# godai0519/BayesianNetwork

Measured on AMD Instinct MI355X. Metric: edge-messages/sec to BP convergence, higher is better.
Workload: dtype f64; 1 GPU; 316x316 2D-grid BN, k=4, 99856 nodes, 199080 edges (BASELINE.json configs[2]), 998 evidence nodes, eps=0.001; parallelism=1 GPU

## Files before the change

### bayesiannetwork_amd/csrc/bn_resident.hip

```cpp
#include "bn_tiles.hpp"

namespace bnmi {

#define RLX_AGENT __ATOMIC_RELAXED, __HIP_MEMORY_SCOPE_AGENT

#ifdef BN_TILE_CLOCK
#define RSTAMP(k, iter, lane_, wave_)                                                              \
    do {                                                                                           \
        if ((iter) == 5 && (lane_) == 0) g_tile_clock[blockIdx.x * kResidentWaves + (wave_)][k] = wall_clock64(); \
    } while (0)
constexpr int kRunClockStamps = 8;
static __device__ unsigned long long g_run_clock[kTileClockTiles][kRunClockStamps];
#define RUNSTAMP(k, lane_, wave_)                                                                   \
    do {                                                                                           \
        if ((lane_) == 0) g_run_clock[blockIdx.x * kResidentWaves + (wave_)][k] = wall_clock64();   \
    } while (0)
#else
#define RSTAMP(k, iter, lane_, wave_) ((void)0)
#define RUNSTAMP(k, lane_, wave_) ((void)0)
#endif

typedef unsigned u32x4 __attribute__((ext_vector_type(4)));
__device__ __forceinline__ double2_t ld_rec(__amdgpu_buffer_rsrc_t r, int64_t idx2) {
    return __builtin_bit_cast(double2_t, __builtin_amdgcn_raw_buffer_load_b128(r, int(idx2) * 16, 0, 16));
}
__device__ __forceinline__ void st_rec(__amdgpu_buffer_rsrc_t r, int64_t idx2, double2_t v) {
    __builtin_amdgcn_raw_buffer_store_b128(__builtin_bit_cast(u32x4, v), r, int(idx2) * 16, 0, 16);
}
__device__ __forceinline__ double2_t ld_rec_sys(__amdgpu_buffer_rsrc_t r, int64_t idx2) {
    return __builtin_bit_cast(double2_t, __builtin_amdgcn_raw_buffer_load_b128(r, int(idx2) * 16, 0, 17));
}
__device__ __forceinline__ void st_rec_sys(__amdgpu_buffer_rsrc_t r, int64_t idx2, double2_t v) {
    __builtin_amdgcn_raw_buffer_store_b128(__builtin_bit_cast(u32x4, v), r, int(idx2) * 16, 0, 17);
}
__device__ __forceinline__ void drain_stores() { asm volatile("s_waitcnt vmcnt(0)" ::: "memory"); }

__device__ __forceinline__ void pin_here(double& x) { asm volatile("" : "+v"(x)); }

#ifndef BN_RES_PRIO
#define BN_RES_PRIO 6
#endif
template <int SCHED, int G>
__device__ __forceinline__ bool prio_segment(int wave) {
    if constexpr (SCHED == 2 || (SCHED == 3 && G < 2)) {
        if (((wave >> 2) & 1) != (G & 1)) __builtin_amdgcn_s_setprio(1);
        else __builtin_amdgcn_s_setprio(0);
        return true;
    } else if constexpr (SCHED == 4) {
        __builtin_amdgcn_s_setprio(3 - G);
        return true;
    } else if constexpr (SCHED == 5 && G != 2) {
        __builtin_amdgcn_s_setprio(G == 0 ? 2 : G == 1 ? 1 : 0);
        return true;
    } else if constexpr (SCHED == 6 && G != 2) {
        if (G == 3 && (wave & 4) == 0) __builtin_amdgcn_s_setprio(0);
        else __builtin_amdgcn_s_setprio(G == 0 ? 3 : G == 1 ? 2 : 1);
        return true;
    }
    return false;
}

struct BlockShared {
    unsigned long long slot[kResidentMaxSets][kResidentWaves];
    int verdict[kResidentMaxSets];
    unsigned long long t_arrive;
    int skew_ticks;
    int arrived[kResidentMaxSets];
    int poll_it[kResidentMaxSets];
    int ver[kResidentMaxSets];
};
enum : int { kGoOn = 0, kConverged = 1, kCapped = 2, kAbort = 3 };

__device__ __forceinline__ double residual_of(unsigned long long bits) {
    const double r = __longlong_as_double((long long)bits);
    return r < DBL_MIN ? DBL_MIN : r;
}
__device__ __forceinline__ int verdict_of(const ResidentArgs& a, double r, int n_done) {
    if (r < a.eps) return kConverged;
    if (a.max_sweeps > 0 && n_done >= a.max_sweeps) return kCapped;
    return kGoOn;
}

__device__ __forceinline__ unsigned long long granule(unsigned gen, unsigned half) { return ((unsigned long long)gen << 32) | half; }

__device__ __forceinline__ void arrive(const ResidentArgs& a, BlockShared& sh, int set, int it, int s, double wres, int lane,
                                       int wave) {
    const unsigned long long bits = wave_umax((unsigned long long)__double_as_longlong(wres));
    if (lane == 0) sh.slot[set][wave] = bits;
    RSTAMP(3, it, lane, wave);
    drain_stores();
    RSTAMP(4, it, lane, wave);
    __syncthreads();
    RSTAMP(5, it, lane, wave);
    if (threadIdx.x == 0) {
        unsigned long long m = 0;
        for (int w = 0; w < a.waves; ++w) m = sh.slot[set][w] > m ? sh.slot[set][w] : m;
        ResidentSync* sy = a.sync + set;
        if (a.n_tile_blocks == 1) {
            sy->res[it] = m;
            sh.verdict[set] = verdict_of(a, residual_of(m), s + 1);
        } else {
            const unsigned gen = a.gen_base + unsigned(it) + 1u;
            unsigned long long* g = (a.direct != 0 && (it & 1)) ? sy->blk_odd[blockIdx.x] : sy->blk[blockIdx.x];
            const unsigned long long now = wall_clock64();
            sh.t_arrive = now;
            __hip_atomic_store(g, granule(gen, unsigned(m >> 32)), RLX_AGENT);
            __hip_atomic_store(g + 1, ((now & 0xffffull) << 48) | ((unsigned long long)(gen & 0xffffu) << 32) | unsigned(m), RLX_AGENT);
        }
    }
}

__device__ __forceinline__ void arrive_batch(const ResidentArgs& a, BlockShared& sh, int set, int it, int s, double wres, int lane, int wave) {
    const unsigned long long bits = wave_umax((unsigned long long)__double_as_longlong(wres));
    if (lane == 0) sh.slot[set][wave] = bits;
    RSTAMP(3, it, lane, wave);
    drain_stores();
    RSTAMP(4, it, lane, wave);
    if (lane == 0) {
        const int before = __hip_atomic_fetch_add(&sh.arrived[set], 1, __ATOMIC_ACQ_REL, __HIP_MEMORY_SCOPE_WORKGROUP);
        if (before == a.waves - 1) {
            __hip_atomic_store(&sh.arrived[set], 0, __ATOMIC_RELAXED, __HIP_MEMORY_SCOPE_WORKGROUP);
            __builtin_amdgcn_fence(__ATOMIC_ACQUIRE, "workgroup");
            unsigned long long m = 0;
            for (int w = 0; w < a.waves; ++w) m = sh.slot[set][w] > m ? sh.slot[set][w] : m;
            ResidentSync* sy = a.sync + set;
            if (a.n_tile_blocks == 1) {
                sy->res[it] = m;
                __hip_atomic_store(&sh.ver[set], it << 2 | verdict_of(a, residual_of(m), s + 1), __ATOMIC_RELEASE, __HIP_MEMORY_SCOPE_WORKGROUP);
            } else {
                const unsigned gen = a.gen_base + unsigned(it) + 1u;
                unsigned long long* g = sy->blk[blockIdx.x];
                const unsigned long long now = wall_clock64();
                __hip_atomic_store(g, granule(gen, unsigned(m >> 32)), RLX_AGENT);
                __hip_atomic_store(g + 1, ((now & 0xffffull) << 48) | ((unsigned long long)(gen & 0xffffu) << 32) | unsigned(m), RLX_AGENT);
            }
        }
    }
    RSTAMP(5, it, lane, wave);
}

template <class Pred>
__device__ __forceinline__ bool poll_until(const ResidentArgs& a, Pred&& pred) {
    const unsigned long long t0 = wall_clock64();
    for (unsigned n = 1;; ++n) {
        if (pred()) return true;
        if ((n & 7u) == 0) {
            if (__hip_atomic_load(&a.sync->abort, RLX_AGENT) != 0) return false;
            if (wall_clock64() - t0 > a.timeout_ticks) {
                if (pred()) return true;
                __hip_atomic_store(&a.sync->abort, 1u, RLX_AGENT);
                return false;
            }
        }
        __builtin_amdgcn_s_sleep(1);
    }
}

__device__ __forceinline__ bool sweep_granules(const unsigned long long* tbl, int lane, int nb, unsigned gen, unsigned long long& acc,
                                               unsigned own16 = 0u, int* late_out = nullptr) {
    static_assert(kResidentMaxBlocks == 4 * kWave, "four pairs per lane cover the table");
    const unsigned voff = unsigned(lane) * 16u;
    u32x4 r0, r1, r2, r3;
    if (nb <= kWave)
        asm volatile("global_load_dwordx4 %0, %1, %2 sc1\n\ts_waitcnt vmcnt(0)" : "=&v"(r0) : "v"(voff), "s"(tbl) : "memory");
    else
        asm volatile("global_load_dwordx4 %0, %4, %5 sc1\n\t"
                     "global_load_dwordx4 %1, %4, %5 offset:1024 sc1\n\t"
                     "global_load_dwordx4 %2, %4, %5 offset:2048 sc1\n\t"
                     "global_load_dwordx4 %3, %4, %5 offset:3072 sc1\n\t"
                     "s_waitcnt vmcnt(0)"
                     : "=&v"(r0), "=&v"(r1), "=&v"(r2), "=&v"(r3) : "v"(voff), "s"(tbl) : "memory");
    bool mine = true;
    acc = 0;
    int late = 0;
    auto take = [&](const u32x4& r, int blk) {
        if (blk < nb) {
            mine = mine && r.y == gen && (r.w & 0xffffu) == (gen & 0xffffu);
            const unsigned long long v = (unsigned long long)r.x << 32 | r.z;
            acc = v > acc ? v : acc;
            const int d = int(short((r.w >> 16) - own16));
            late = d > late ? d : late;
        }
    };
    take(r0, lane);
    if (nb > kWave) { take(r1, lane + kWave); take(r2, lane + 2 * kWave); take(r3, lane + 3 * kWave); }
    if (late_out) *late_out = late;
    return mine;
}

__device__ __forceinline__ int wait_verdict(const ResidentArgs& a, BlockShared& sh, int set, int it) {
    if (a.direct != 0 && a.n_tile_blocks > 1) {
        if (threadIdx.x < kWave) {
            int lane = int(threadIdx.x);
            asm volatile("" : "+v"(lane));
            ResidentSync* sy = a.sync + set;
            const unsigned gen = a.gen_base + unsigned(it) + 1u;
            const int nb = a.n_tile_blocks;
            const unsigned long long* tbl = (it & 1) ? &sy->blk_odd[0][0] : &sy->blk[0][0];
            unsigned long long m = 0;
            const unsigned long long t_arr = sh.t_arrive;
            const unsigned own16 = unsigned(t_arr) & 0xffffu;
            if (a.first_poll_delay >= 0) {
                const unsigned long long first_at = t_arr + (unsigned long long)(sh.skew_ticks + a.first_poll_delay);
                while (wall_clock64() < first_at) __builtin_amdgcn_s_sleep(1);
            }
            int late = 0;
            const bool ok = poll_until(a, [&] { return __all(sweep_granules(tbl, lane, nb, gen, m, own16, &late)) != 0; });
            m = wave_umax(m);
            {
                int mx = late;
#pragma unroll
                for (int off = 32; off >= 1; off >>= 1) { const int o = __shfl_xor(mx, off, kWave); mx = o > mx ? o : mx; }
                if (lane == 0) sh.skew_ticks = ok ? (mx < 400 ? mx : 400) : 0;
            }
            if (lane == 0) {
                if (blockIdx.x == 0 && ok) __hip_atomic_store(&sy->res[it], m, RLX_AGENT);
                sh.verdict[set] = ok ? verdict_of(a, residual_of(m), a.sweep_begin + it + 1) : kAbort;
            }
        }
        __syncthreads();
        return sh.verdict[set];
    }
    if (threadIdx.x == 0 && a.n_tile_blocks > 1) {
        ResidentSync* sy = a.sync + set;
        const unsigned gen = a.gen_base + unsigned(it) + 1u;
        const int groups = a.n_tile_blocks < 8 ? a.n_tile_blocks : 8;
        const int g = blockIdx.x % groups;
        unsigned word = 0;
        const bool ok = poll_until(a, [&] {
            word = __hip_atomic_load(&sy->grp[g].gen, RLX_AGENT);
            return (word & 0x3fffffffu) >= gen;
        });
        sh.verdict[set] = ok ? int(word >> 30) : kAbort;
    }
    __syncthreads();
    return sh.verdict[set];
}

__device__ __forceinline__ int wait_verdict_batch(const ResidentArgs& a, BlockShared& sh, int set, int it, int lane) {
    int out = __hip_atomic_load(&sh.ver[set], __ATOMIC_ACQUIRE, __HIP_MEMORY_SCOPE_WORKGROUP);
    if ((out >> 2) == it) return out & 3;
    int before = it;
    if (lane == 0) before = __hip_atomic_fetch_max(&sh.poll_it[set], it, __ATOMIC_ACQ_REL, __HIP_MEMORY_SCOPE_WORKGROUP);
    if (__builtin_amdgcn_readfirstlane(before) < it && a.n_tile_blocks > 1) {
        if (lane == 0) {
            ResidentSync* sy = a.sync + set;
            const unsigned gen = a.gen_base + unsigned(it) + 1u;
            const int groups = a.n_tile_blocks < 8 ? a.n_tile_blocks : 8;
            const int g = blockIdx.x % groups;
            unsigned word = 0;
            const bool ok = poll_until(a, [&] {
                word = __hip_atomic_load(&sy->grp[g].gen, RLX_AGENT);
                return (word & 0x3fffffffu) >= gen;
            });
            __hip_atomic_store(&sh.ver[set], it << 2 | (ok ? int(word >> 30) : kAbort), __ATOMIC_RELEASE, __HIP_MEMORY_SCOPE_WORKGROUP);
        }
    }
    const unsigned long long t0 = wall_clock64();
    for (unsigned n = 1; ((out = __hip_atomic_load(&sh.ver[set], __ATOMIC_ACQUIRE, __HIP_MEMORY_SCOPE_WORKGROUP)) >> 2) != it; ++n) {
        if ((n & 63u) == 0 && wall_clock64() - t0 > 2 * a.timeout_ticks) {
            __hip_atomic_store(&a.sync->abort, 1u, RLX_AGENT);
            return kAbort;
        }
        __builtin_amdgcn_s_sleep(1);
    }
    return out & 3;
}

__device__ __forceinline__ void resident_service(const ResidentArgs& a, int lane) {
    if (a.direct != 0) return;
    const int nb = a.n_tile_blocks;
    const int groups = nb < 8 ? nb : 8;
    unsigned active = a.set_mask;
    for (int it = 0; it < a.budget; ++it) {
        const unsigned gen = a.gen_base + unsigned(it) + 1u;
        for (int set = 0; set < a.n_sets; ++set) {
            if (((active >> set) & 1u) == 0) continue;
            ResidentSync* sy = a.sync + set;
            unsigned long long m = 0;
            if (!poll_until(a, [&] { return __all(sweep_granules(&sy->blk[0][0], lane, nb, gen, m)) != 0; }))
                return;
            m = wave_umax(m);
            const int verdict = verdict_of(a, residual_of(m), a.sweep_begin + it + 1);
            if (lane == 0) {
                __hip_atomic_store(&sy->res[it], m, RLX_AGENT);
                asm volatile("s_waitcnt vmcnt(0)" ::: "memory");
                const unsigned word = gen | (unsigned(verdict) << 30);
                for (int q = 0; q < groups; ++q) __hip_atomic_store(&sy->grp[q].gen, word, RLX_AGENT);
            }
            if (verdict != kGoOn) active &= ~(1u << set);
        }
        if (active == 0) break;
    }
}

template <bool BATCH, class Phase, class Finalize>
__device__ __forceinline__ bool resident_drive(const ResidentArgs& a, BlockShared& sh, int lane, int wave, Phase&& phase,
                                               Finalize&& finalize) {
    unsigned active = BATCH ? a.set_mask : 1u;
    const int n_sets = BATCH ? a.n_sets : 1;
    for (int it = 0; it <= a.budget; ++it) {
        const int s = a.sweep_begin + it;
        for (int set = 0; set < n_sets; ++set) {
            if (((active >> set) & 1u) == 0) continue;
            int v = kGoOn;
            RSTAMP(0, it, lane, wave);
            if (it > 0) {
                if (BATCH && a.direct == 0) v = wait_verdict_batch(a, sh, set, it - 1, lane);
                else v = wait_verdict(a, sh, set, it - 1);
                if (v == kAbort) return false;
            }
            RSTAMP(1, it, lane, wave);
            if (v != kGoOn || it == a.budget) {
                const int done = v != kGoOn ? v : 0;
                RUNSTAMP(4, lane, wave);
                finalize(set, s, done, true);
                RUNSTAMP(5, lane, wave);
                if (blockIdx.x == 0 && wave == 0) {
                    const ResidentSync* sy = a.sync + set;
                    double* hist = a.b.res_hist + int64_t(set) * a.res_hist_stride;
                    int q0 = lane;
                    asm volatile("" : "+v"(q0));
                    for (int q = q0; q < it; q += kWave)
                        if (a.sweep_begin + q < a.b.res_cap)
                            hist[a.sweep_begin + q] = residual_of(__hip_atomic_load(&sy->res[q], RLX_AGENT));
                    if (lane == 0) {
                        Ctl* hc = a.host_ctl + set;
                        hc->last_res = it > 0 ? residual_of(__hip_atomic_load(&sy->res[it - 1], RLX_AGENT)) : 0.0;
                        hc->n_sweeps = s;
                        hc->run_id = a.run_id;
                        hc->done = done;
                    }
                }
                active &= ~(1u << set);
                continue;
            }
            const double wres = phase(set, s);
            if (BATCH && a.direct == 0) arrive_batch(a, sh, set, it, s, wres, lane, wave);
            else arrive(a, sh, set, it, s, wres, lane, wave);
            RSTAMP(6, it, lane, wave);
            if (it == 0) RUNSTAMP(3, lane, wave);
        }
        if (active == 0) break;
    }
    return true;
}

template <bool BATCH>
__device__ __forceinline__ bool resident_idle(const ResidentArgs& a, BlockShared& sh, int lane, int wave) {
    return resident_drive<BATCH>(a, sh, lane, wave, [](int, int) { return 0.0; }, [](int, int, int, bool) {});
}

#define RLX_SYS __ATOMIC_RELAXED, __HIP_MEMORY_SCOPE_SYSTEM
template <bool SHARD>
__device__ __forceinline__ unsigned long long flow_load(const unsigned long long* p) {
    if constexpr (SHARD) return __hip_atomic_load(p, RLX_SYS);
    else return __hip_atomic_load(p, RLX_AGENT);
}
template <bool SHARD>
__device__ __forceinline__ void flow_store(unsigned long long* p, unsigned long long v) {
    if constexpr (SHARD) __hip_atomic_store(p, v, RLX_SYS);
    else __hip_atomic_store(p, v, RLX_AGENT);
}
__device__ __forceinline__ unsigned long long* flow_slot(FlowSync* f, int nranks, int par, int slot) {
    return reinterpret_cast<unsigned long long*>(f + 1) + (size_t(par) * nranks * kFlowSlotsPerRank + slot) * 2;
}

template <bool SHARD>
__device__ __forceinline__ void flow_raise_abort(const ResidentArgs& a, unsigned where = 0) {
    const unsigned long long w = (unsigned long long)(a.gen_base + 1u) | ((unsigned long long)kFlowAbort << 32);
    for (int q = 0; q < 8; ++q) flow_store<SHARD>(&a.flow->verdict[q].word, w);
    if constexpr (SHARD) {
        for (int r = 0; r < a.b.nranks; ++r)
            if (r != a.b.rank)
                for (int q = 0; q < 8; ++q) flow_store<true>(&a.peers[r].flow->verdict[q].word, w);
    }
    __hip_atomic_store(a.host_abort, 0x80000000u | where, __ATOMIC_RELAXED, __HIP_MEMORY_SCOPE_SYSTEM);
}

template <bool SHARD>
__device__ __forceinline__ unsigned flow_wait(const ResidentArgs& a, int tile, int it, int lane, int& n_it) {
    n_it = 0;
    if (it == 0) return kFlowGoOn;
    FlowSync* f = a.flow;
    const int32_t* nbr_list = a.nbr + int64_t(tile) * a.nbr_chunks * kWave + lane;
    int round = 0;
    int nbr = nbr_list[0];
    const unsigned long long* vword = &f->verdict[blockIdx.x & 7].word;
    const unsigned want_nb = a.gen_base + unsigned(it);
    const unsigned want_v = a.gen_base + unsigned(it) - 1u;
    unsigned long long t0 = 0;
    for (unsigned polls = 0;; ++polls) {
        bool nb_ok = true;
        if (nbr >= 0) nb_ok = unsigned(flow_load<SHARD>(flow_slot(f, a.b.nranks, (it - 1) & 1, nbr)) >> 32) == want_nb;
        if (__all(nb_ok) && round + 1 < a.nbr_chunks) {
            ++round;
            nbr = nbr_list[round * kWave];
            if (__any(nbr >= 0)) continue;
        }
        const unsigned long long w = flow_load<SHARD>(vword);
        const unsigned gen = unsigned(w), kind = unsigned(w >> 32);
        const bool ours = gen - (a.gen_base + 1u) < unsigned(kResidentBudget);
        if (ours && kind != kFlowGoOn) {
            n_it = int(gen - a.gen_base);
            return kind;
        }
        const bool v_ok = it < 2 || (ours && gen >= want_v);
        if (it < a.budget && v_ok && __all(nb_ok)) return kFlowGoOn;
        if ((polls & 31u) == 31u) {
            const unsigned long long now = wall_clock64();
            if (t0 == 0) t0 = now;
            if (now - t0 > a.timeout_ticks) {
                if (lane == 0) flow_raise_abort<SHARD>(a, 1u | (unsigned(it) << 8) | (unsigned(tile) << 20));
                return kFlowAbort;
            }
        }
        for (int z = 0; z < a.poll_sleep; ++z) __builtin_amdgcn_s_sleep(8);
    }
}

template <bool SHARD, class Phase, class Finalize>
__device__ __forceinline__ bool flow_drive(const ResidentArgs& a, int tile, int lane, int wave, Phase&& phase, Finalize&& finalize) {
    const int my_slot = a.b.rank * kFlowSlotsPerRank + tile;
    unsigned pub = 0;
    if constexpr (SHARD) pub = a.pub_mask[tile];
    for (int it = 0;; ++it) {
        RSTAMP(0, it, lane, wave);
        int n_it;
        const unsigned v = flow_wait<SHARD>(a, tile, it, lane, n_it);
        RSTAMP(1, it, lane, wave);
        if (v == kFlowAbort) return false;
        if (v != kFlowGoOn) {
            RUNSTAMP(4, lane, wave);
            finalize(0, a.sweep_begin + n_it, v == kFlowBudget ? 0 : int(v), n_it == it);
            RUNSTAMP(5, lane, wave);
            return true;
        }
        const double wres = phase(0, a.sweep_begin + it);
        const unsigned long long bits = wave_umax((unsigned long long)__double_as_longlong(wres));
        RSTAMP(3, it, lane, wave);
        drain_stores();
        RSTAMP(4, it, lane, wave);
        const unsigned gen = a.gen_base + unsigned(it) + 1u;
        if (lane == 0) {
            unsigned long long* g = flow_slot(a.flow, a.b.nranks, it & 1, my_slot);
            flow_store<SHARD>(g, granule(gen, unsigned(bits >> 32)));
            flow_store<SHARD>(g + 1, granule(gen, unsigned(bits)));
        }
        if constexpr (SHARD) {
            const int q = lane - 1;
            if (q >= 0 && q < a.b.nranks && ((pub >> q) & 1u) != 0) {
                unsigned long long* g = flow_slot(a.peers[q].flow, a.b.nranks, it & 1, my_slot);
                flow_store<true>(g, granule(gen, 0u));
            }
        }
        RSTAMP(6, it, lane, wave);
        if (it == 0) RUNSTAMP(3, lane, wave);
    }
}

template <bool SHARD>
__device__ __forceinline__ void flow_service(const ResidentArgs& a, BlockShared& sh, int lane, int wave) {
    FlowSync* f = a.flow;
    const int nt = a.b.n_tiles, nranks = a.b.nranks, base = a.b.rank * kFlowSlotsPerRank;
    const unsigned long long t_first = wall_clock64();
    if (threadIdx.x == 0) sh.verdict[1] = 0;
    __syncthreads();
    int n_it = 0;
    unsigned v = kFlowGoOn;
    for (int it = 0; it < a.budget; ++it) {
        const unsigned gen = a.gen_base + unsigned(it) + 1u;
        unsigned long long m = 0;
        unsigned long long t0 = 0;
        bool ok = true;
        for (unsigned polls = 0;; ++polls) {
            bool mine = true;
            unsigned long long acc = 0;
            for (int t = threadIdx.x; t < nt; t += a.waves * kWave) {
                const unsigned long long* g = flow_slot(f, nranks, it & 1, base + t);
                const unsigned long long hi = flow_load<SHARD>(g);
                const unsigned long long lo = flow_load<SHARD>(g + 1);
                mine = mine && unsigned(hi >> 32) == gen && unsigned(lo >> 32) == gen;
                const unsigned long long x = (hi << 32) | (lo & 0xffffffffull);
                acc = x > acc ? x : acc;
            }
            m = acc;
            if (__all(mine)) break;
            const unsigned long long w = flow_load<SHARD>(&f->verdict[0].word);
            if (unsigned(w >> 32) == kFlowAbort && unsigned(w) - (a.gen_base + 1u) < unsigned(kResidentBudget)) { ok = false; break; }
            if ((polls & 31u) == 31u) {
                const unsigned long long now = wall_clock64();
                if (t0 == 0) t0 = now;
                if (now - t0 > a.timeout_ticks) {
                    if (lane == 0) flow_raise_abort<SHARD>(a, 2u | (unsigned(it) << 8));
                    ok = false;
                    break;
                }
            }
            __builtin_amdgcn_s_sleep(1);
        }
        m = wave_umax(m);
        if (lane == 0) {
            sh.slot[0][wave] = m;
            if (!ok) sh.verdict[1] = 1;
        }
        __syncthreads();
        if (threadIdx.x == 0) {
            unsigned decision = kFlowAbort;
            bool good = sh.verdict[1] == 0;
            unsigned long long mm = 0;
            if (good) {
                for (int w = 0; w < a.waves; ++w) mm = sh.slot[0][w] > mm ? sh.slot[0][w] : mm;
            }
            if constexpr (SHARD) {
                if (good) {
                    for (int r = 0; r < nranks; ++r) {
                        unsigned long long* g = &a.peers[r].flow->rank_granule[it & 1][a.b.rank][0];
                        flow_store<true>(g, granule(gen, unsigned(mm >> 32)));
                        flow_store<true>(g + 1, granule(gen, unsigned(mm)));
                    }
                    unsigned long long t1 = 0;
                    for (unsigned polls = 0; good; ++polls) {
                        bool all = true;
                        unsigned long long acc = 0;
                        for (int r = 0; r < nranks; ++r) {
                            const unsigned long long hi = flow_load<true>(&f->rank_granule[it & 1][r][0]);
                            const unsigned long long lo = flow_load<true>(&f->rank_granule[it & 1][r][1]);
                            all = all && unsigned(hi >> 32) == gen && unsigned(lo >> 32) == gen;
                            const unsigned long long x = (hi << 32) | (lo & 0xffffffffull);
                            acc = x > acc ? x : acc;
                        }
                        if (all) { mm = acc; break; }
                        const unsigned long long w = flow_load<true>(&f->verdict[0].word);
                        if (unsigned(w >> 32) == kFlowAbort && unsigned(w) - (a.gen_base + 1u) < unsigned(kResidentBudget)) good = false;
                        if ((polls & 31u) == 31u) {
                            const unsigned long long now = wall_clock64();
                            if (t1 == 0) t1 = now;
                            if (now - t1 > a.timeout_ticks) {
                                flow_raise_abort<true>(a, 3u | (unsigned(it) << 8));
                                good = false;
                            }
                        }
                        __builtin_amdgcn_s_sleep(1);
                    }
                }
            }
            if (good) {
                decision = unsigned(verdict_of(a, residual_of(mm), a.sweep_begin + it + 1));
                if (decision == kFlowGoOn && it == a.budget - 1) decision = kFlowBudget;
                flow_store<SHARD>(&f->res[it], mm);
                asm volatile("s_waitcnt vmcnt(0)" ::: "memory");
                const unsigned long long word = (unsigned long long)gen | ((unsigned long long)decision << 32);
                for (int q = 0; q < 8; ++q) flow_store<SHARD>(&f->verdict[q].word, word);
            }
            sh.verdict[0] = int(decision);
        }
        __syncthreads();
        v = unsigned(sh.verdict[0]);
        n_it = it + 1;
        if (v != kFlowGoOn) break;
    }
    if (wave != 0) return;
    if (v != kFlowAbort) {
        double* hist = a.b.res_hist;
        for (int q = lane; q < n_it; q += kWave)
            if (a.sweep_begin + q < a.b.res_cap) hist[a.sweep_begin + q] = residual_of(flow_load<SHARD>(&f->res[q]));
    }
    if (lane == 0) {
        Ctl* hc = a.host_ctl;
        hc->last_res = (v != kFlowAbort && n_it > 0) ? residual_of(flow_load<SHARD>(&f->res[n_it - 1])) : 0.0;
        hc->n_sweeps = a.sweep_begin + n_it;
        hc->t_first = t_first;
        hc->t_last = wall_clock64();
        hc->run_id = a.run_id;
        hc->done = v == kFlowAbort ? -1 : (v == kFlowBudget ? 0 : int(v));
    }
}

template <int K, int M, int RC, bool BATCH, bool FLOW, bool SHARD = false, bool BIG = false, bool UNI = false>
__device__ __forceinline__ bool resident_tile(const ResidentArgs& a, BlockShared& sh, const TileDesc& td, int tile, int lane, int wave,
                                              double2_t* cpt_lds) {
    static_assert(!(BATCH && FLOW), "the dataflow form runs one evidence set");
    static_assert(!SHARD || FLOW, "shards exchange through the dataflow form");
    constexpr int KP = (K + 1) & ~1, H = KP / 2;
    constexpr int C = ipow(K, M), S = K * C, SP = (S + 1) & ~1;
    constexpr int CB = (M > 0) ? C / K : 0;
    constexpr int SR = (S > 32 && !BIG) ? 28 : SP;
    static_assert(SR % 2 == 0 && (SR == SP || (S - SR) / 2 <= kResidentLdsSlots), "CPT split");
    auto PIN = [](double& x) { if constexpr (!BIG) pin_here(x); };
    constexpr int kPrio = (!BATCH && !FLOW && !BIG) ? BN_RES_PRIO : 0;
    const BpBuffers& b = a.b;
    const bool active = lane < td.n_nodes;
    const int lc = active ? lane : 0;

    const double2_t* cp = reinterpret_cast<const double2_t*>(b.cpt + td.cpt_base) + lc;
    double cpt[SR];
#pragma unroll
    for (int q = 0; q < SR / 2; ++q) {
        const double2_t x = cp[q * kWave];
        cpt[2 * q] = x.x;
        cpt[2 * q + 1] = x.y;
    }
    RUNSTAMP(1, lane, wave);
    if constexpr (SR < SP) {
#pragma unroll
        for (int q = SR / 2; q < S / 2; ++q) cpt_lds[(q - SR / 2) * kWave + lane] = cp[q * kWave];
    }
#ifdef BN_TILE_CLOCK
    asm volatile("s_waitcnt vmcnt(0) lgkmcnt(0)" ::: "memory");
    RUNSTAMP(2, lane, wave);
#endif
    bool frozen = false;
    const int64_t rbase = td.rec_base / 2 + lc;
    const MsgRef* orf = b.out_refs + td.out_base + lc;
    const bool btile = SHARD && tile >= a.n_interior;
    const bool in_by_ref = SHARD && td.in_ref_base >= 0;
    auto IREF = [&](int j) -> MsgRef { return b.in_refs[td.in_ref_base + j * kWave + lc]; };
    auto in_idx = [&](int j, int part, int h) -> int64_t {
        if constexpr (SHARD) {
            if (in_by_ref) {
                const MsgRef r = IREF(j);
                const bool cut = r.lam < 0;
                const int lam = cut ? ~r.lam : r.lam;
                const int stride = cut ? 1 : (lam - r.pi) / H;
                return int64_t((part ? lam : r.pi) + h * stride);
            }
        }
        return rbase + ((j * 2 + part) * H + h) * kWave;
    };
    auto LD = [&](__amdgpu_buffer_rsrc_t r, int64_t idx2) -> double2_t {
        if constexpr (SHARD) {
            if (btile) return ld_rec_sys(r, idx2);
        }
        return ld_rec(r, idx2);
    };
    auto ST = [&](__amdgpu_buffer_rsrc_t r, int64_t idx2, double2_t v) {
        if constexpr (SHARD) {
            if (btile) { st_rec_sys(r, idx2, v); return; }
        }
        st_rec(r, idx2, v);
    };
    auto push_remote = [&](bool cut_lane, int64_t other, bool into_rec1, const int64_t (&idx)[H], const double2_t (&val)[H]) {
        if constexpr (SHARD) {
            if (!btile) return;
            for (int q = 0; q < b.nranks; ++q) {
                if (q == b.rank) continue;
                const int64_t lo = b.g_base + int64_t(q) * b.seg_d2;
                const bool mine = cut_lane && other >= lo && other < lo + b.seg_d2;
                if (__any(mine)) {
                    double* base = into_rec1 ? a.peers[q].rec1 : a.peers[q].rec0;
                    const __amdgpu_buffer_rsrc_t pr = __builtin_amdgcn_make_buffer_rsrc(base, 0, int(a.peers[q].rec_bytes), 0x00020000);
                    const int64_t shift = a.peers[q].g_base - b.g_base;
                    if (mine) {
#pragma unroll
                        for (int h = 0; h < H; ++h) st_rec_sys(pr, idx[h] + shift, val[h]);
                    }
                }
            }
        }
    };
    constexpr bool kRefsResident = RC <= 4;
    MsgRef oref[RC > 0 ? RC : 1];
#pragma unroll
    for (int c = 0; c < RC; ++c) {
        oref[c] = MsgRef{-1, 0};
        if (kRefsResident && active && c < td.cmax) oref[c] = orf[c * kWave];
    }
    double piv[KP], lav[KP];
    auto load_nodes = [&](int set, int s) {
        frozen = b.frozen[(BATCH ? int64_t(set) * a.slot_stride : 0) + td.slot_base + lc] == b.frozen_mark;
#pragma unroll
        for (int i = 0; i < KP; ++i) {
            piv[i] = (M == 0 && i < K) ? cpt[i] : 1.0;
            lav[i] = 1.0;
        }
        if (frozen || s > 0) {
            const double* nodd = b.node1;
            if constexpr (!BATCH && !FLOW) {
                if (s == 1) {
                    if (const Memo0Image* mi = a.memo) nodd = mi->node;
                }
            }
            const double2_t* nin = reinterpret_cast<const double2_t*>(((s & 1) ? nodd : b.node0) + (BATCH ? int64_t(set) * a.node_stride : 0) +
                                                                      td.node_base) + lc;
#pragma unroll
            for (int h = 0; h < H; ++h) {
                const double2_t x = nin[h * kWave], y = nin[(H + h) * kWave];
                piv[2 * h] = x.x; piv[2 * h + 1] = x.y;
                lav[2 * h] = y.x; lav[2 * h + 1] = y.y;
            }
        }
    };
    auto store_nodes = [&](int set, int n) {
        if (!active) return;
        double2_t* nout = reinterpret_cast<double2_t*>(((n & 1) ? b.node1 : b.node0) + (BATCH ? int64_t(set) * a.node_stride : 0) + td.node_base) + lane;
#pragma unroll
        for (int h = 0; h < H; ++h) {
            double2_t y, z;
            y.x = piv[2 * h]; y.y = (2 * h + 1 < K) ? piv[2 * h + 1] : 0.0;
            z.x = lav[2 * h]; z.y = (2 * h + 1 < K) ? lav[2 * h + 1] : 0.0;
            nout[h * kWave] = y;
            nout[(H + h) * kWave] = z;
        }
    };
    if constexpr (!BATCH) load_nodes(0, a.sweep_begin);

    const size_t rec_bytes = size_t(b.rec_total_doubles) * 8;
    auto phase = [&](int set, int s) -> double {
        if constexpr (BATCH) load_nodes(set, s);
        if constexpr (kPrio >= 2) prio_segment<kPrio, 0>(wave);
        const bool first = s == 0;
        const __amdgpu_buffer_rsrc_t rsrc0 = __builtin_amdgcn_make_buffer_rsrc(b.rec0 + (BATCH ? int64_t(set) * a.rec_stride : 0), 0, int(rec_bytes), 0x00020000);
        double* rodd = b.rec1 + (BATCH ? int64_t(set) * a.rec_stride : 0);
        if constexpr (!BATCH && !FLOW) {
            if (s == 1) {
                if (const Memo0Image* mi = a.memo) rodd = mi->rec;
            }
        }
        const __amdgpu_buffer_rsrc_t rsrc1 = __builtin_amdgcn_make_buffer_rsrc(rodd, 0, int(rec_bytes), 0x00020000);
        const __amdgpu_buffer_rsrc_t rin = (s & 1) ? rsrc1 : rsrc0;
        const __amdgpu_buffer_rsrc_t rout = (s & 1) ? rsrc0 : rsrc1;

        double wres = 0.0;
        double lan[K];
        {
            if constexpr (!kRefsResident) {
#pragma unroll
                for (int c = 0; c < RC; ++c) {
                    oref[c] = MsgRef{-1, 0};
                    if (active && c < td.cmax) oref[c] = orf[c * kWave];
                }
            }
            double lkc[RC > 0 ? RC : 1][KP];
#pragma unroll
            for (int c = 0; c < RC; ++c)
#pragma unroll
                for (int i = 0; i < KP; ++i) lkc[c][i] = 1.0;
            if (!first) {
#pragma unroll
                for (int c = 0; c < RC; ++c)
                    if (c < td.cmax) {
                        const Loc l = decode_ref(oref[c], H);
#pragma unroll
                        for (int h = 0; h < H; ++h) {
                            const double2_t y = LD(rin, l.lam + h * l.stride);
                            lkc[c][2 * h] = l.has ? y.x : 1.0;
                            lkc[c][2 * h + 1] = l.has ? y.y : 1.0;
                        }
                    }
            }
#pragma unroll
            for (int i = 0; i < K; ++i) {
                double acc = 1.0;
#pragma unroll
                for (int c = 0; c < RC; ++c) acc *= lkc[c][i];
                lan[i] = acc;
            }
            normalize_k<K>(lan);
#pragma unroll
            for (int c = 0; c < RC; ++c) {
                if (c < td.cmax) {
                    PIN(wres);
#pragma unroll
                    for (int i = 0; i < K; ++i) PIN(piv[i]);

                    double u[K];
#pragma unroll
                    for (int i = 0; i < K; ++i) {
                        double acc = piv[i];
#pragma unroll
                        for (int x = 0; x < RC; ++x)
                            if (x != c) acc *= lkc[x][i];
                        u[i] = acc;
                    }
                    normalize_k<K>(u);
                    const Loc l = decode_ref(oref[c], H);
                    if (l.has) {
                        double old[KP], o[KP];
#pragma unroll
                        for (int i = 0; i < KP; ++i) { old[i] = 1.0; o[i] = 0.0; }
                        if (!first) {
#pragma unroll
                            for (int h = 0; h < H; ++h) {
                                const double2_t x = LD(rin, l.pi + h * l.stride);
                                old[2 * h] = x.x; old[2 * h + 1] = x.y;
                            }
                        }
#pragma unroll
                        for (int i = 0; i < K; ++i) {
                            o[i] = u[i];
                            wres = res_acc(wres, fabs(u[i] - old[i]));
                        }
                        int64_t at[H];
                        double2_t yv[H];
#pragma unroll
                        for (int h = 0; h < H; ++h) {
                            yv[h].x = o[2 * h]; yv[h].y = o[2 * h + 1];
                            at[h] = l.pi + h * l.stride;
                            ST(rout, at[h], yv[h]);
                        }
                        if constexpr (SHARD) push_remote(oref[c].lam < 0, l.lam, (s & 1) == 0, at, yv);
                    }
                }
            }
        }

        RSTAMP(7, s - a.sweep_begin, lane, wave);
        __builtin_amdgcn_sched_barrier(0);
        if constexpr (kPrio >= 2) {
            if (prio_segment<kPrio, 1>(wave)) __builtin_amdgcn_sched_barrier(0);
        }
        double pim[M > 0 ? M : 1][KP];
#pragma unroll
        for (int j = 0; j < M; ++j)
#pragma unroll
            for (int i = 0; i < KP; ++i) pim[j][i] = 1.0;
        if (!first) {
#pragma unroll
            for (int j = 0; j < M; ++j)
#pragma unroll
                for (int h = 0; h < H; ++h) {
                    const double2_t x = LD(rin, in_idx(j, 0, h));
                    pim[j][2 * h] = x.x; pim[j][2 * h + 1] = x.y;
                }
        }
        double pin[K];
        double out[M > 0 ? M : 1][K];
#pragma unroll
        for (int jt = 0; jt < M; ++jt)
#pragma unroll
            for (int ct = 0; ct < K; ++ct) out[jt][ct] = 0.0;
#pragma unroll
        for (int ib = 0; ib < K; ++ib) {
            if constexpr (M == 0) {
                pin[ib] = 0.0 + cpt[ib];
            } else {
                if constexpr (kPrio >= 2) {
                    if (ib == K / 2) prio_segment<kPrio, 2>(wave);
                }
                PIN(lav[ib]);
#pragma unroll
                for (int j = 0; j < M; ++j)
#pragma unroll
                    for (int i = 0; i < K; ++i) PIN(pim[j][i]);
#pragma unroll
                for (int jt = 0; jt < M; ++jt)
#pragma unroll
                    for (int ct = 0; ct < K; ++ct) PIN(out[jt][ct]);
                const double* lds_lane = reinterpret_cast<const double*>(cpt_lds + lane);
                auto ROW = [&](int cond) -> double {
                    const int e = ib * C + cond;
                    if (e < SR) return cpt[e < SR ? e : 0];
                    return lds_lane[((e - SR) >> 1) * (2 * kWave) + (e & 1)];
                };
                double acc = 0.0;
#pragma unroll
                for (int rr = 0; rr < CB; ++rr) {
                    if (rr > 0) {
                        if constexpr (!BIG) asm volatile("" ::: "memory");
                        PIN(acc);
                        PIN(lav[ib]);
#pragma unroll
                        for (int j = 0; j < M; ++j)
#pragma unroll
                            for (int i = 0; i < K; ++i) PIN(pim[j][i]);
#pragma unroll
                        for (int jt = 0; jt < M; ++jt)
#pragma unroll
                            for (int ct = 0; ct < K; ++ct) PIN(out[jt][ct]);
                    }
                    if constexpr (M == 2 && !SHARD) {
#pragma unroll
                        for (int x = 0; x < K; ++x) {
                            const double r = ROW(rr * K + x);
                            double value = r * pim[0][rr];
                            value *= pim[1][x];
                            acc += value;
                            const double t = lav[ib] * r;
                            out[0][rr] += t * pim[1][x];
                            out[1][x] += t * pim[0][rr];
                        }
                        continue;
                    }
#pragma unroll
                    for (int x = 0; x < K; ++x) {
                        const int cond = rr * K + x;
                        double value = ROW(cond);
#pragma unroll
                        for (int j = 0; j < M; ++j) value *= pim[j][(cond / ipow(K, M - 1 - j)) % K];
                        acc += value;
                    }
#pragma unroll
                    for (int jt = 0; jt < M; ++jt) {
                        const int stride = ipow(K, M - 1 - jt);
#pragma unroll
                        for (int ct = 0; ct < K; ++ct) {
                            const int cond = (rr / stride) * stride * K + ct * stride + (rr % stride);
                            double value = lav[ib] * ROW(cond);
#pragma unroll
                            for (int j = 0; j < M; ++j)
                                if (j != jt) value *= pim[j][(cond / ipow(K, M - 1 - j)) % K];
                            out[jt][ct] += value;
                        }
                    }
                }
                pin[ib] = acc;
            }
        }
        RSTAMP(8, s - a.sweep_begin, lane, wave);
        __builtin_amdgcn_sched_barrier(0);
        if constexpr (kPrio >= 2) {
            if (prio_segment<kPrio, 3>(wave)) __builtin_amdgcn_sched_barrier(0);
        }
        normalize_k<K>(pin);
#pragma unroll
        for (int jt = 0; jt < M; ++jt) normalize_k<K>(out[jt]);

#pragma unroll
        for (int jt = 0; jt < M; ++jt) {
            double old[KP], o[KP];
#pragma unroll
            for (int i = 0; i < KP; ++i) { old[i] = 1.0; o[i] = 0.0; }
            if (!first) {
#pragma unroll
                for (int h = 0; h < H; ++h) {
                    const double2_t y = LD(rin, in_idx(jt, 1, h));
                    old[2 * h] = y.x; old[2 * h + 1] = y.y;
                }
            }
#pragma unroll
            for (int i = 0; i < K; ++i) {
                o[i] = out[jt][i];
                wres = res_acc(wres, fabs(out[jt][i] - old[i]));
            }
            if (active) {
                int64_t at[H];
                double2_t yv[H];
#pragma unroll
                for (int h = 0; h < H; ++h) {
                    yv[h].x = o[2 * h]; yv[h].y = o[2 * h + 1];
                    at[h] = in_idx(jt, 1, h);
                    ST(rout, at[h], yv[h]);
                }
                if constexpr (SHARD) {
                    if (in_by_ref) {
                        const MsgRef r = IREF(jt);
                        push_remote(r.lam < 0, r.pi, (s & 1) == 0, at, yv);
                    }
                }
            }
        }
        if (!active) wres = 0.0;
        if (!frozen) {
#pragma unroll
            for (int i = 0; i < K; ++i) { piv[i] = pin[i]; lav[i] = lan[i]; }
        }
        if constexpr (BATCH || FLOW) store_nodes(set, s + 1);
        if constexpr (kPrio >= 2) __builtin_amdgcn_s_setprio(0);
        return wres;
    };
    auto finalize = [&](int set, int n, int done, bool regs_hold_n) {
        if constexpr (BATCH) load_nodes(set, n);
        else if constexpr (FLOW) { if (!regs_hold_n) load_nodes(set, n); }
        else store_nodes(set, n);
        if (active && done != 0) {
            const int64_t boff = b.slot_boff[td.slot_base + lane];
            double* beliefs = b.beliefs + (BATCH ? int64_t(set) * a.belief_stride : 0);
            double bel[K];
            double sum = 0;
#pragma unroll
            for (int i = 0; i < K; ++i) {
                bel[i] = piv[i] * lav[i];
                sum += bel[i];
            }
            if constexpr (UNI && K % 2 == 0) {
                double2_t* b2 = reinterpret_cast<double2_t*>(beliefs + boff);
#pragma unroll
                for (int h = 0; h < K / 2; ++h) {
                    double2_t y;
                    y.x = bel[2 * h] / sum;
                    y.y = bel[2 * h + 1] / sum;
                    b2[h] = y;
                }
            } else {
#pragma unroll
                for (int i = 0; i < K; ++i) beliefs[boff + i] = bel[i] / sum;
            }
        }
    };
    if constexpr (kPrio == 1) {
        if (wave & 4) __builtin_amdgcn_s_setprio(1);
    }
    if constexpr (FLOW) return flow_drive<SHARD>(a, tile, lane, wave, phase, finalize);
    else return resident_drive<BATCH>(a, sh, lane, wave, phase, finalize);
}

enum : int { kModeBarrier = 0, kModeBatch = 1, kModeFlow = 2, kModeFlowShard = 3 };

template <int K, int M, int MODE, int LEAN, bool BIG>
__device__ __forceinline__ bool resident_dispatch(const ResidentArgs& a, BlockShared& sh, const TileDesc& td, int tile, int lane, int wave,
                                                  double2_t* cpt_lds) {
    constexpr bool BATCH = MODE == kModeBatch, FLOW = MODE == kModeFlow || MODE == kModeFlowShard, SHARD = MODE == kModeFlowShard;
#ifdef BN_RES_ONLY_RC
    return resident_tile<K, M, BN_RES_ONLY_RC, BATCH, FLOW, SHARD, BIG>(a, sh, td, tile, lane, wave, cpt_lds);
#else
    if constexpr (LEAN != 0) return resident_tile<K, M, 2, BATCH, FLOW, SHARD, BIG, true>(a, sh, td, tile, lane, wave, cpt_lds);
    if (td.cmax <= 2) return resident_tile<K, M, 2, BATCH, FLOW, SHARD, BIG>(a, sh, td, tile, lane, wave, cpt_lds);
    if (td.cmax <= 4) return resident_tile<K, M, 4, BATCH, FLOW, SHARD, BIG>(a, sh, td, tile, lane, wave, cpt_lds);
    return resident_tile<K, M, 8, BATCH, FLOW, SHARD, BIG>(a, sh, td, tile, lane, wave, cpt_lds);
#endif
}

template <int MODE, int LEAN, int WMAX = kResidentWaves>
__global__ __launch_bounds__(WMAX * kWave, WMAX == kResidentWaves ? 2 : 1) void bp_resident_kernel(ResidentArgs a) {
    constexpr bool BATCH = MODE == kModeBatch, FLOW = MODE == kModeFlow || MODE == kModeFlowShard, SHARD = MODE == kModeFlowShard;
    __shared__ BlockShared sh;
    __shared__ double2_t cpt_lds_all[WMAX][kResidentLdsSlots * kWave];
    const BpBuffers& b = a.b;
    const int lane = threadIdx.x & (kWave - 1);
    const int wave = __builtin_amdgcn_readfirstlane(threadIdx.x >> 6);
    if (threadIdx.x == 0) { sh.t_arrive = 0; sh.skew_ticks = 0; }
    if constexpr (BATCH) {
        if (threadIdx.x < kResidentMaxSets) { sh.arrived[threadIdx.x] = 0; sh.poll_it[threadIdx.x] = -1; sh.ver[threadIdx.x] = -1; }
        __syncthreads();
    }
    if constexpr (!FLOW) {
        if (blockIdx.x == 0 && threadIdx.x == 0) {
            const unsigned long long t_first = wall_clock64();
            for (int set = 0; set < a.n_sets; ++set) a.host_ctl[set].t_first = t_first;
            if constexpr (MODE == kModeBarrier) {
                if (a.n_tile_blocks == 1) {
                    if (const Memo0Image* mi = a.memo) {
                        if (mi->word_before != nullptr) b.res_hist[-1] = residual_of(*mi->word_before);
                    }
                }
            }
        }
    }
    if (int(blockIdx.x) < a.n_tile_blocks) RUNSTAMP(0, lane, wave);
    const int nb = a.n_tile_blocks;
    if (int(blockIdx.x) >= nb) {
        if constexpr (MODE == kModeBarrier) {
            if (threadIdx.x == 0) {
                if (const Memo0Image* mi = a.memo) {
                    if (mi->word_before != nullptr) b.res_hist[-1] = residual_of(*mi->word_before);
                }
            }
        }
        if constexpr (FLOW) flow_service<SHARD>(a, sh, lane, wave);
        else if (wave == 0) resident_service(a, lane);
        return;
    }
    const int lb = (nb % 8 == 0) ? (blockIdx.x & 7) * (nb >> 3) + (blockIdx.x >> 3) : blockIdx.x;
    const int tile = lb * a.waves + wave;
    bool ok;
    if (tile >= b.n_tiles) {
        if constexpr (FLOW) return;
        else ok = resident_idle<BATCH>(a, sh, lane, wave);
    } else {
        const TileDesc td = b.tiles[tile];
        double2_t* lds = cpt_lds_all[wave];
        {
#ifdef BN_RES_ONLY_K
            ok = resident_dispatch<BN_RES_ONLY_K, BN_RES_ONLY_M, MODE, LEAN, (WMAX < kResidentWaves)>(a, sh, td, tile, lane, wave, lds);
#else
            if constexpr (LEAN != 0) {
                switch (td.m) {
                    case 0: ok = resident_dispatch<LEAN, 0, MODE, LEAN, (WMAX < kResidentWaves)>(a, sh, td, tile, lane, wave, lds); break;
                    case 1: ok = resident_dispatch<LEAN, 1, MODE, LEAN, (WMAX < kResidentWaves)>(a, sh, td, tile, lane, wave, lds); break;
                    default: ok = resident_dispatch<LEAN, 2, MODE, LEAN, (WMAX < kResidentWaves)>(a, sh, td, tile, lane, wave, lds); break;
                }
            } else {
                switch (td.kv * 8 + td.m) {
                    case 2 * 8 + 0: ok = resident_dispatch<2, 0, MODE, 0, (WMAX < kResidentWaves)>(a, sh, td, tile, lane, wave, lds); break;
                    case 2 * 8 + 1: ok = resident_dispatch<2, 1, MODE, 0, (WMAX < kResidentWaves)>(a, sh, td, tile, lane, wave, lds); break;
                    case 2 * 8 + 2: ok = resident_dispatch<2, 2, MODE, 0, (WMAX < kResidentWaves)>(a, sh, td, tile, lane, wave, lds); break;
                    case 3 * 8 + 0: ok = resident_dispatch<3, 0, MODE, 0, (WMAX < kResidentWaves)>(a, sh, td, tile, lane, wave, lds); break;
                    case 3 * 8 + 1: ok = resident_dispatch<3, 1, MODE, 0, (WMAX < kResidentWaves)>(a, sh, td, tile, lane, wave, lds); break;
                    case 3 * 8 + 2: ok = resident_dispatch<3, 2, MODE, 0, (WMAX < kResidentWaves)>(a, sh, td, tile, lane, wave, lds); break;
                    case 4 * 8 + 0: ok = resident_dispatch<4, 0, MODE, 0, (WMAX < kResidentWaves)>(a, sh, td, tile, lane, wave, lds); break;
                    case 4 * 8 + 1: ok = resident_dispatch<4, 1, MODE, 0, (WMAX < kResidentWaves)>(a, sh, td, tile, lane, wave, lds); break;
                    default: ok = resident_dispatch<4, 2, MODE, 0, (WMAX < kResidentWaves)>(a, sh, td, tile, lane, wave, lds); break;
                }
            }
#endif
        }
    }
    if constexpr (MODE == kModeBarrier) {
        if (blockIdx.x == 0 && threadIdx.x == 0) {
            if (const Memo0Image* mi = a.memo) {
                if (b.res_cap > 0) b.res_hist[0] = residual_of(*mi->word);
            }
        }
    }
    if constexpr (!FLOW) {
        if (!ok && threadIdx.x == 0 && a.host_abort) __hip_atomic_store(a.host_abort, 1u, __ATOMIC_RELAXED, __HIP_MEMORY_SCOPE_SYSTEM);
        if (blockIdx.x == 0 && threadIdx.x == 0) {
            const unsigned long long t_last = wall_clock64();
            for (int set = 0; set < a.n_sets; ++set) {
                a.host_ctl[set].t_last = t_last;
                if (!ok) { a.host_ctl[set].run_id = a.run_id; a.host_ctl[set].done = -1; }
            }
        }
    }
}

int launch_bp_resident(const ResidentArgs& a, int grid_blocks, int lean_k, void* stream) {
    (void)hipGetLastError();
    const dim3 g(grid_blocks), t(a.waves * kWave);
    hipStream_t s = (hipStream_t)stream;
    const int mode = a.n_sets > 1 ? kModeBatch : (a.flow != nullptr ? (a.peers != nullptr ? kModeFlowShard : kModeFlow) : kModeBarrier);
#define BN_RES_LAUNCH(L)                                                                          \
    switch (mode) {                                                                               \
        case kModeBatch: hipLaunchKernelGGL((bp_resident_kernel<kModeBatch, L>), g, t, 0, s, a); break;   \
        case kModeFlow: hipLaunchKernelGGL((bp_resident_kernel<kModeFlow, L>), g, t, 0, s, a); break;     \
        case kModeFlowShard: hipLaunchKernelGGL((bp_resident_kernel<kModeFlowShard, L>), g, t, 0, s, a); break; \
        default: hipLaunchKernelGGL((bp_resident_kernel<kModeBarrier, L>), g, t, 0, s, a); break;         \
    }
#define BN_RES_LAUNCH_W4(L)                                                                       \
    switch (mode) {                                                                               \
        case kModeBatch: hipLaunchKernelGGL((bp_resident_kernel<kModeBatch, L, 4>), g, t, 0, s, a); break;   \
        case kModeFlow: hipLaunchKernelGGL((bp_resident_kernel<kModeFlow, L, 4>), g, t, 0, s, a); break;     \
        case kModeFlowShard: hipLaunchKernelGGL((bp_resident_kernel<kModeFlowShard, L, 4>), g, t, 0, s, a); break; \
        default: hipLaunchKernelGGL((bp_resident_kernel<kModeBarrier, L, 4>), g, t, 0, s, a); break;         \
    }
    const bool w4 = a.waves <= 4 && grid_blocks > 1;
    switch (lean_k) {
        case 2: BN_RES_LAUNCH(2); break;
        case 3: BN_RES_LAUNCH(3); break;
        case 4: if (w4) { BN_RES_LAUNCH_W4(4); } else { BN_RES_LAUNCH(4); } break;
        default: if (w4) { BN_RES_LAUNCH_W4(0); } else { BN_RES_LAUNCH(0); } break;
    }
#undef BN_RES_LAUNCH_W4
#undef BN_RES_LAUNCH
    hipError_t e = hipGetLastError();
    return e == hipSuccess ? 0 : int(e);
}

}

#ifdef BN_TILE_CLOCK
extern "C" int bn_debug_run_clock_resident(unsigned long long* out, int n_waves) {
    if (n_waves > bnmi::kTileClockTiles) n_waves = bnmi::kTileClockTiles;
    return int(hipMemcpyFromSymbol(out, HIP_SYMBOL(bnmi::g_run_clock), sizeof(unsigned long long) * bnmi::kRunClockStamps * n_waves));
}
extern "C" int bn_debug_tile_clock_resident(unsigned long long* out, int n_tiles) {
    if (n_tiles > bnmi::kTileClockTiles) n_tiles = bnmi::kTileClockTiles;
    return int(hipMemcpyFromSymbol(out, HIP_SYMBOL(bnmi::g_tile_clock), sizeof(unsigned long long) * bnmi::kTileClockStamps * n_tiles));
}
#endif
```

Baseline: 40.24 billion edge-messages/s.

## Shorten the verdict critical path by offloading residual recording to an idle wave

The converged/continue verdict now comes from a per-lane __all test against eps, so the full 64-lane max reduction no longer sits on the critical path. The residual-history store is moved to an idle wave in the last partial block (ResidualRecorder), which re-sweeps the granule table off the critical path. The skew estimate is now kept per lane in LDS and reduced with a bitwise __any search. This spreads work across more waves and may cost extra memory traffic from the recorder's second sweep.

```diff
diff --git a/bayesiannetwork_amd/csrc/bn_resident.hip b/bayesiannetwork_amd/csrc/bn_resident.hip
--- a/bayesiannetwork_amd/csrc/bn_resident.hip
+++ b/bayesiannetwork_amd/csrc/bn_resident.hip
@@ -64,10 +64,11 @@
     unsigned long long slot[kResidentMaxSets][kResidentWaves];
     int verdict[kResidentMaxSets];
     unsigned long long t_arrive;
-    int skew_ticks;
+    int block_reports;
     int arrived[kResidentMaxSets];
     int poll_it[kResidentMaxSets];
     int ver[kResidentMaxSets];
+    int late[kWave];
 };
 enum : int { kGoOn = 0, kConverged = 1, kCapped = 2, kAbort = 3 };
 
@@ -188,6 +189,10 @@
     return mine;
 }
 
+__device__ __forceinline__ bool has_recorder(const ResidentArgs& a) {
+    return a.direct != 0 && a.n_tile_blocks > 1 && (a.b.n_tiles & (a.waves - 1)) != 0;
+}
+
 __device__ __forceinline__ int wait_verdict(const ResidentArgs& a, BlockShared& sh, int set, int it) {
     if (a.direct != 0 && a.n_tile_blocks > 1) {
         if (threadIdx.x < kWave) {
@@ -201,21 +206,29 @@
             const unsigned long long t_arr = sh.t_arrive;
             const unsigned own16 = unsigned(t_arr) & 0xffffu;
             if (a.first_poll_delay >= 0) {
-                const unsigned long long first_at = t_arr + (unsigned long long)(sh.skew_ticks + a.first_poll_delay);
+                const int prev = sh.late[lane];
+                int skew = 0;
+                if (__any(prev >= 400)) skew = 400;
+                else {
+#pragma unroll
+                    for (int bit = 256; bit >= 1; bit >>= 1)
+                        if (__any(prev >= (skew | bit))) skew |= bit;
+                }
+                const unsigned long long first_at = t_arr + (unsigned long long)(skew + a.first_poll_delay);
                 while (wall_clock64() < first_at) __builtin_amdgcn_s_sleep(1);
             }
             int late = 0;
             const bool ok = poll_until(a, [&] { return __all(sweep_granules(tbl, lane, nb, gen, m, own16, &late)) != 0; });
-            m = wave_umax(m);
-            {
-                int mx = late;
-#pragma unroll
-                for (int off = 32; off >= 1; off >>= 1) { const int o = __shfl_xor(mx, off, kWave); mx = o > mx ? o : mx; }
-                if (lane == 0) sh.skew_ticks = ok ? (mx < 400 ? mx : 400) : 0;
-            }
-            if (lane == 0) {
-                if (blockIdx.x == 0 && ok) __hip_atomic_store(&sy->res[it], m, RLX_AGENT);
-                sh.verdict[set] = ok ? verdict_of(a, residual_of(m), a.sweep_begin + it + 1) : kAbort;
+            RSTAMP(2, it + 1, lane, 0);
+            const bool below = residual_of(m) < a.eps;
+            const int n_done = a.sweep_begin + it + 1;
+            const int v = !ok ? kAbort : __all(below) ? kConverged : (a.max_sweeps > 0 && n_done >= a.max_sweeps) ? kCapped : kGoOn;
+            if (lane == 0) sh.verdict[set] = v;
+            RSTAMP(9, it + 1, lane, 0);
+            sh.late[lane] = ok ? late : 0;
+            if (blockIdx.x == 0 && ok && sh.block_reports != 0) {
+                m = wave_umax(m);
+                if (lane == 0) __hip_atomic_store(&sy->res[it], m, RLX_AGENT);
             }
         }
         __syncthreads();
@@ -294,9 +307,36 @@
     }
 }
 
-template <bool BATCH, class Phase, class Finalize>
+struct NoRecorder {
+    __device__ __forceinline__ void operator()(const ResidentArgs&, int, int, int) const {}
+    __device__ __forceinline__ bool reports(const BlockShared& sh, int wave) const { return wave == 0 && sh.block_reports != 0; }
+};
+struct ResidualRecorder {
+    bool on;
+    __device__ __forceinline__ void operator()(const ResidentArgs& a, int set, int it, int lane) const {
+        if (!on) return;
+        ResidentSync* sy = a.sync + set;
+        const unsigned long long* tbl = (it & 1) ? &sy->blk_odd[0][0] : &sy->blk[0][0];
+        unsigned long long m = 0;
+        const bool same = __all(sweep_granules(tbl, lane, a.n_tile_blocks, a.gen_base + unsigned(it) + 1u, m)) != 0;
+#ifdef BN_TILE_CLOCK
+        if (!same && lane == 0) {
+            unsigned long long& bad = g_run_clock[blockIdx.x * kResidentWaves + (threadIdx.x >> 6)][6];
+            if (bad == 0) bad = (unsigned long long)it + 1;
+        }
+#else
+        (void)same;
+#endif
+        m = wave_umax(m);
+        if (lane == 0) __hip_atomic_store(&sy->res[it], m, RLX_AGENT);
+        drain_stores();
+    }
+    __device__ __forceinline__ bool reports(const BlockShared&, int) const { return on; }
+};
+
+template <bool BATCH, class Phase, class Finalize, class Record = NoRecorder>
 __device__ __forceinline__ bool resident_drive(const ResidentArgs& a, BlockShared& sh, int lane, int wave, Phase&& phase,
-                                               Finalize&& finalize) {
+                                               Finalize&& finalize, Record record = Record()) {
     unsigned active = BATCH ? a.set_mask : 1u;
     const int n_sets = BATCH ? a.n_sets : 1;
     for (int it = 0; it <= a.budget; ++it) {
@@ -309,6 +349,7 @@
                 if (BATCH && a.direct == 0) v = wait_verdict_batch(a, sh, set, it - 1, lane);
                 else v = wait_verdict(a, sh, set, it - 1);
                 if (v == kAbort) return false;
+                record(a, set, it - 1, lane);
             }
             RSTAMP(1, it, lane, wave);
             if (v != kGoOn || it == a.budget) {
@@ -316,7 +357,7 @@
                 RUNSTAMP(4, lane, wave);
                 finalize(set, s, done, true);
                 RUNSTAMP(5, lane, wave);
-                if (blockIdx.x == 0 && wave == 0) {
+                if (record.reports(sh, wave)) {
                     const ResidentSync* sy = a.sync + set;
                     double* hist = a.b.res_hist + int64_t(set) * a.res_hist_stride;
                     int q0 = lane;
@@ -347,8 +388,9 @@
 }
 
 template <bool BATCH>
-__device__ __forceinline__ bool resident_idle(const ResidentArgs& a, BlockShared& sh, int lane, int wave) {
-    return resident_drive<BATCH>(a, sh, lane, wave, [](int, int) { return 0.0; }, [](int, int, int, bool) {});
+__device__ __forceinline__ bool resident_idle(const ResidentArgs& a, BlockShared& sh, int lane, int wave, int tile) {
+    const ResidualRecorder record{!BATCH && has_recorder(a) && tile == a.b.n_tiles};
+    return resident_drive<BATCH>(a, sh, lane, wave, [](int, int) { return 0.0; }, [](int, int, int, bool) {}, record);
 }
 
 #define RLX_SYS __ATOMIC_RELAXED, __HIP_MEMORY_SCOPE_SYSTEM
@@ -1019,7 +1061,13 @@
     const BpBuffers& b = a.b;
     const int lane = threadIdx.x & (kWave - 1);
     const int wave = __builtin_amdgcn_readfirstlane(threadIdx.x >> 6);
-    if (threadIdx.x == 0) { sh.t_arrive = 0; sh.skew_ticks = 0; }
+    if (threadIdx.x == 0) {
+        sh.t_arrive = 0;
+        sh.block_reports = (!FLOW && blockIdx.x == 0 && !has_recorder(a)) ? 1 : 0;
+    }
+    if constexpr (!FLOW) {
+        if (threadIdx.x < kWave) sh.late[threadIdx.x] = 0;
+    }
     if constexpr (BATCH) {
         if (threadIdx.x < kResidentMaxSets) { sh.arrived[threadIdx.x] = 0; sh.poll_it[threadIdx.x] = -1; sh.ver[threadIdx.x] = -1; }
         __syncthreads();
@@ -1056,7 +1104,7 @@
     bool ok;
     if (tile >= b.n_tiles) {
         if constexpr (FLOW) return;
-        else ok = resident_idle<BATCH>(a, sh, lane, wave);
+        else ok = resident_idle<BATCH>(a, sh, lane, wave, tile);
     } else {
         const TileDesc td = b.tiles[tile];
         double2_t* lds = cpt_lds_all[wave];
```

Result: faster. 41.96 billion edge-messages/s (median of 6 runs) (+4.3%).
